# 3DAnimals/3DAnimals

Hardware: AMD Instinct MI355X
Metric: train images/sec fwd+bwd @256x256 b16 (higher is better)
Workload: dtype f32

## Files before the change

3danimals_amd/_lib.py:

```python
from __future__ import annotations

import ctypes
import os

import torch

_HERE = os.path.dirname(os.path.abspath(__file__))
LIB_PATH = os.environ.get("A3D_LIB") or os.path.join(_HERE, "lib", "liba3d_hip.so")

_c_int, _c_float, _c_size_t, _p = ctypes.c_int, ctypes.c_float, ctypes.c_size_t, ctypes.c_void_p

SIGNATURES = {
    "a3d_version": (_c_int, []),
    "a3d_last_error": (ctypes.c_char_p, []),
    "a3d_bw_probe_fill": (_c_int, [_p, ctypes.c_int64, _p]),
    "a3d_bw_probe_read": (_c_int, [_p, ctypes.c_int64, _p, _p]),
    "a3d_dmtet_scratch_bytes": (_c_size_t, [_c_int, _c_int]),
    "a3d_dmtet_count": (_c_int, [_p, _p, _p, _c_int, _c_int, _p, _p, _p, _c_int, _c_int, _p, _p, _c_int, _p, _c_int, _p]),
    "a3d_dmtet_count_ordered": (_c_int, [_p, _c_int, _c_int, _c_int, _p, _p, _p, _p, _c_int, _p, _c_int, _p]),
    "a3d_dmtet_word_group_slots": (_c_int, []),
    "a3d_dmtet_word_group_bits": (_c_int, []),
    "a3d_dmtet_block_items": (_c_int, []),
    "a3d_dmtet_vertex_scratch_bytes": (_c_size_t, [_c_int]),
    "a3d_dmtet_gather_rows": (_c_int, [_p, _p, ctypes.c_int64, ctypes.c_int64, _c_int, _p, _p]),
    "a3d_dmtet_emit": (_c_int, [_p, _p, _p, _p, _c_int, _c_int, _p, _c_int, _c_int, _c_int, _p, _p, _p, _p, _p, _p]),
    "a3d_dmtet_emit_sparse": (_c_int, [_p, _p, _p, _p, _c_int, _c_int, _p, _c_int, _c_int, _c_int, _p, _p, _p, _p, _p, _p]),
    "a3d_dmtet_bwd": (_c_int, [_p, _p, _p, _p, _p, _c_int, _c_int, _p, _p, _c_int, _p]),
    "a3d_skin_fwd": (_c_int, [_p, _c_int, _p, _c_int, _p, _c_int, _c_int, _c_int, _c_float, _p, _p, _p, _p]),
    "a3d_skin_bwd": (_c_int, [_p, _p, _c_int, _p, _c_int, _p, _c_int, _c_int, _c_int, _c_float, _p, _p, _c_int, _p]),
    "a3d_bone_transforms_fwd": (_c_int, [_p, _c_int, _p, _p, _c_int, _c_int, _c_int, _p, _p]),
    "a3d_bone_transforms_bwd": (_c_int, [_p, _p, _c_int, _p, _p, _c_int, _c_int, _c_int, _p, _p]),
    "a3d_estimate_bones": (_c_int, [_p, _p]),
    "a3d_skin_pose_max_bones": (_c_int, []),
    "a3d_skin_pose_products_floats": (_c_size_t, [_c_int, _c_int]),
    "a3d_skin_pose_fwd": (_c_int, [_p, _c_int, _p, _c_int, _p, _p, _c_int, _c_int, _c_int, _c_int, _c_float, _p, _p, _p, _p, _p]),
    "a3d_skin_pose_bwd": (_c_int, [_p, _p, _c_int, _p, _c_int, _p, _p, _p, _p, _c_int, _c_int, _c_int, _c_int, _c_float, _p, _p, _p, _c_int, _p]),
    "a3d_normals_adjacency": (_c_int, [_p, _c_int, _c_int, _p, _p, _p, _p]),
    "a3d_normals_fwd": (_c_int, [_p, _p, _p, _p, _c_int, _c_int, _c_int, _p, _p, _c_int, _p]),
    "a3d_normals_fwd_pair": (_c_int, [_p, _c_int, _p, _c_int, _p, _p, _p, _c_int, _c_int, _p, _p, _p, _p, _c_int, _p]),
    "a3d_normals_bwd": (_c_int, [_p, _c_int, _p, _p, _p, _p, _p, _c_int, _c_int, _c_int, _p, _p, _c_int, _p, _p]),
    "a3d_shade_fwd": (_c_int, [_p, _p, _c_int, _p, _p, _c_int, ctypes.c_int64, _c_int, _p, _p, _p, _p, _c_int, _p]),
    "a3d_shade_bwd": (_c_int, [_p, _p, _p, _p, _p, _c_int, _p, _c_int, _p, _c_int, ctypes.c_int64, _c_int, _p, _p, _p, _c_int, _p]),
    "a3d_shade_bwd_rows": (_c_int, [_p, _p, _p, _p, _p, ctypes.c_int64, _p, _c_int, ctypes.c_int64, _c_int, _p, _p, _c_int, ctypes.c_int64, _p]),
    "a3d_xfm_points_fwd": (_c_int, [_p, _c_int, _p, _c_int, _c_int, _c_int, _p, _p, _p]),
    "a3d_flow_delta_fwd": (_c_int, [_p, _c_int, _c_int, _c_int, _p, _p]),
    "a3d_flow_delta_bwd": (_c_int, [_p, _c_int, _p, _c_int, _c_int, _c_int, _p, _p]),
    "a3d_xfm_points_bwd": (_c_int, [_p, _c_int, _p, _c_int, _p, _c_int, _c_int, _c_int, _p, _p, _c_int, _p, _c_int, _p, _c_int, _p, _c_int, _p]),
    "a3d_cover_scratch_bytes": (_c_size_t, [_c_int, _c_int, _c_int]),
    "a3d_cover_blocks": (_c_int, [_c_int, _c_int, _c_int]),
    "a3d_cover_groups": (_c_int, [_c_int, _c_int, _c_int]),
    "a3d_cover_group_stride": (_c_int, []),
    "a3d_cover_count": (_c_int, [_p, _c_int, _c_int, _c_int, _c_int, _p, _p]),
    "a3d_cover_emit": (_c_int, [_p, _c_int, _c_int, _c_int, _c_int, _p, _p, _p, _p]),
    "a3d_rast_scratch_bytes": (_c_size_t, [_c_int, _c_int, _c_int]),
    "a3d_rast_bins_bytes": (_c_size_t, [_c_int, _c_int, _c_int, _c_int]),
    "a3d_rast_resolve": (_c_int, [_p, _c_int, _p, _c_int, _c_int, _c_int, _c_int, _c_int, _p, _p, _p, _p]),
    "a3d_rast_resolve_gbuffer_fwd": (_c_int, [_p, _c_int, _p, _c_int, _c_int, _c_int, _c_int, _c_int, _p, _p, _p, ctypes.c_int64, _p, _p, _p, _p, _p,
                                              _c_int, _p, _p, _c_int, _p, _p, _p, _p]),
    "a3d_rast_fwd": (_c_int, [_p, _c_int, _p, _c_int, _c_int, _c_int, _c_int, _c_int, _p, _p, _c_int, _p, _p]),
    "a3d_dispatch_order_probe": (_c_int, [_c_int, _c_int, _p, _p]),
    "a3d_rast_bwd": (_c_int, [_p, _p, _p, _c_int, _p, _c_int, _c_int, _c_int, _c_int, _c_int, _p, _p]),
    "a3d_interp_fwd": (_c_int, [_p, _c_int, _c_int, _p, _p, _c_int, _c_int, _c_int, _c_int, _c_int, _p, _p]),
    "a3d_interp_bwd": (_c_int, [_p, _p, _c_int, _c_int, _p, _p, _c_int, _c_int, _c_int, _c_int, _c_int, _p, _p, _p]),
    "a3d_mesh_topology": (_c_int, [_p, _c_int, _c_int, _p, _p, _p, _p, _p, _c_int, _p]),
    "a3d_mesh_topology_finalize_max_vertices": (_c_int, []),
    "a3d_mesh_topology_finalize": (_c_int, [_p, _c_int, _c_int, _p, _p, _p, _p, _c_int, _p]),
    "a3d_gbuffer_fwd": (_c_int, [_p, _p, _p, ctypes.c_int64, _p, _p, _p, _c_int, _c_int, _c_int, _c_int, _c_int, _c_int, _p, _p, _c_int, _p, _p, _p, _p]),
    "a3d_cover_gbuffer_fwd": (_c_int, [_p, _p, _c_int, _c_int, _c_int, _c_int, _c_int, _p, ctypes.c_int64, _p, _p, _p, _p, _p, _c_int, _p, _p, _c_int,
                                       _p, _p, _p, _p]),
    "a3d_gbuffer_bwd": (_c_int, [_p, _p, _p, _p, ctypes.c_int64, _p, _p, _p, _c_int, _p, _c_int, _c_int, _c_int, _c_int, _c_int, _p, _c_int,
                                 _c_int, _p, _c_int, _p, _p, _p]),
    "a3d_gbuffer_prior_grad": (_c_int, [_p, _c_int, _c_int, _p, _p]),
    "a3d_gemm_nn_relumask": (_c_int, [_p, _p, _p, ctypes.c_int64, _c_int, _c_int, _p, _p]),
    "a3d_harmonic_embed_fwd": (_c_int, [_p, _p, _c_int, _c_int, _c_int, ctypes.c_int64, _p, _p]),
    "a3d_harmonic_embed_bwd": (_c_int, [_p, _p, _p, _c_int, _c_int, _c_int, ctypes.c_int64, _p, _p]),
    "a3d_recon_losses_scratch_bytes": (_c_size_t, [_c_int, _c_int, _c_int]),
    "a3d_recon_losses_mask_bytes": (_c_size_t, [_c_int, _c_int, _c_int]),
    "a3d_recon_losses_columns": (_c_int, []),
    "a3d_recon_losses_fwd": (_c_int, [_p, _p, _c_int, _c_int, _p, _p, _p, _p, _p, ctypes.c_int64, _p, _c_int, _c_int, _c_int, _p, _p, _p, _p]),
    "a3d_recon_losses_bwd": (_c_int, [_p, _p, _p, _c_int, _c_int, _c_int, _p, _p, _p, _p, _p, ctypes.c_int64, _p, _c_int, _c_int, _c_int, _p, _p, _p, _p]),
    "a3d_flow_loss_scratch_bytes": (_c_size_t, [_c_int, _c_int, _c_int, _c_int]),
    "a3d_flow_loss_fwd": (_c_int, [_p, _c_int, _p, _p, _c_int, _c_int, _c_int, _c_int, _p, _p, _p, _p]),
    "a3d_flow_loss_bwd": (_c_int, [_p, _p, _p, _c_int, _p, _p, _c_int, _c_int, _c_int, _c_int, _p, _p]),
    "a3d_rows_segsum": (_c_int, [_p, _p, ctypes.c_int64, _c_int, _c_int, _p, _p]),
    "a3d_rows_add_relu_fwd": (_c_int, [_p, _p, _p, ctypes.c_int64, _c_int, _c_int, _p]),
    "a3d_rows_add_relu_bwd": (_c_int, [_p, _p, _p, ctypes.c_int64, _c_int, _c_int, _p, _p, _p]),
    "a3d_aa_hash_bytes": (_c_size_t, [_c_int]),
    "a3d_aa_shards": (_c_int, []),
    "a3d_aa_capacity": (_c_int, [_c_int, _c_int, _c_int]),
    "a3d_aa_topology": (_c_int, [_p, _c_int, _c_int, _p, _p, _p]),
    "a3d_aa_topology_from_lists": (_c_int, [_p, _c_int, _p, _p, _p, _c_int, _p]),
    "a3d_aa_analyze": (_c_int, [_p, _p, _c_int, _p, _p, _c_int, _c_int, _c_int, _c_int, _c_int, _p, _p, _c_int, _p, _c_int, _p, _p, _c_int, _p]),
    "a3d_aa_fwd": (_c_int, [_p, _c_int, _p, _p, _c_int, _c_int, _c_int, _c_int, _p, _p]),
    "a3d_aa_bwd": (_c_int, [_p, _p, _c_int, _p, _p, _c_int, _p, _c_int, _p, _c_int, _c_int, _c_int, _c_int, _c_int, _p, _p, _p]),
    "a3d_composite_aa_fwd": (_c_int, [_p, _p, _p, _p, _p, _c_int, _c_int, _c_int, _c_int, _p, _p, _p]),
    "a3d_mask_aa_fwd": (_c_int, [_p, _c_int, _p, _c_int, _p, _p, _p, _c_int, _c_int, _c_int, _c_int, _p, _p]),
    "a3d_mask_aa_bwd": (_c_int, [_p, _p, _c_int, _p, _c_int, _p, _p, _c_int, _p, _c_int, _p, _c_int, _c_int, _c_int, _c_int, _c_int, _p, _c_int, _p]),
    "a3d_composite_aa_bwd": (_c_int, [_p, _p, _p, ctypes.c_int64, _p, _p, _p, _c_int, _p, _c_int, _p, _c_int, _c_int, _c_int, _c_int, _c_int, _p, _p, _p]),
}



class DmtetOrder(ctypes.Structure):

    _fields_ = [("size", ctypes.c_uint32), ("group_slots", ctypes.c_int32), ("vertex_of_rank", _p), ("edges_ranked", _p), ("edge_of_row", _p),
                ("tets_ranked", _p), ("tet_of_row", _p), ("edge_groups", _p), ("tet_groups", _p)]


class RastOpts(ctypes.Structure):

    _fields_ = [("size", ctypes.c_uint32), ("lists_stride", ctypes.c_int32), ("prev_rast", _p), ("cover_scratch", _p), ("aa_screen", _p),
                ("aa_count", _p), ("topo_off", _p), ("topo_adj", _p), ("topo_opp", _p), ("normals_v_a", _p), ("normals_v_b", _p),
                ("normals_off", _p), ("normals_adj", _p), ("normals_acc_a", _p), ("normals_a", _p), ("normals_acc_b", _p), ("normals_b", _p),
                ("normals_B_a", ctypes.c_int32), ("normals_B_b", ctypes.c_int32), ("bins", _p), ("bin_cap", ctypes.c_int32), ("bins_clean", ctypes.c_int32),
                ("defer_resolve", ctypes.c_int32), ("reserved", ctypes.c_int32)]


class AaRide(ctypes.Structure):

    _fields_ = [("size", ctypes.c_uint32), ("clip_batch", ctypes.c_int32), ("rast", _p), ("screen", _p), ("tri", _p), ("opp", _p), ("off", _p),
                ("adj", _p), ("V", ctypes.c_int32), ("F", ctypes.c_int32), ("lists_stride", ctypes.c_int32), ("reserved", ctypes.c_int32)]


class CaBuffer(ctypes.Structure):

    _fields_ = [("size", ctypes.c_uint32), ("C", ctypes.c_int32), ("vals", _p), ("bg", _p), ("out", _p), ("g_out", _p), ("g_vals", _p),
# ... 346 lines not shown
```

3danimals_amd/csrc/build.py:

```python
import os
import subprocess
import sys
from concurrent.futures import ThreadPoolExecutor

HERE = os.path.dirname(os.path.abspath(__file__))
PKG = os.path.dirname(HERE)
LIB_DIR = os.path.join(PKG, "lib")
LIB = os.path.join(LIB_DIR, "liba3d_hip.so")
OBJ_DIR = os.path.join(HERE, "build")

SOURCES = {
    "common.hip": [],
    "dmtet.hip": ["-ffp-contract=off"],
    "skin.hip": [],
    "bones.hip": [],
    "normals.hip": ["-ffp-contract=off"],
    "raster.hip": ["-ffp-contract=off"],
    "cover.hip": [],
    "shade.hip": ["-ffp-contract=off"],
    "interp.hip": [],
    "gbuffer.hip": [],
    "segsum.hip": [],
    "losses.hip": [],
    "embed.hip": ["-ffp-contract=off"],
    "gemm.hip": [],
    "antialias.hip": ["-ffp-contract=off"],
    "topology.hip": [],
    "xfm.hip": ["-ffp-contract=off"],
}
COMMON = ["--offload-arch=gfx950", "-O3", "-std=c++17", "-fPIC", "-fhip-fp32-correctly-rounded-divide-sqrt", "-Wall",
          "-Wno-unused-function"]


def _hipcc():
    for c in (os.environ.get("HIPCC"), "/opt/rocm/bin/hipcc", "hipcc"):
        if c and (os.path.isabs(c) and os.path.exists(c) or not os.path.isabs(c)):
            return c
    raise RuntimeError("hipcc not found")


def _stale(target, deps):
    if not os.path.exists(target):
        return True
    t = os.path.getmtime(target)
    return any(os.path.getmtime(d) > t for d in deps)


def build(force=False, verbose=True, profile=False, exp=False):
    assert not (profile and exp)
    lib = os.path.join(LIB_DIR, "liba3d_hip_prof.so") if profile else (os.path.join(LIB_DIR, "liba3d_hip_exp.so") if exp else LIB)
    obj_dir = os.path.join(OBJ_DIR, "prof") if profile else (os.path.join(OBJ_DIR, "exp") if exp else OBJ_DIR)
    os.makedirs(LIB_DIR, exist_ok=True)
    os.makedirs(obj_dir, exist_ok=True)
    hipcc = _hipcc()
    headers = sorted(os.path.join(HERE, f) for f in os.listdir(HERE) if f.endswith(".h")) + [os.path.join(os.path.dirname(PKG), "include", "a3d.h"), os.path.abspath(__file__)]
    jobs = []
    objs = []
    for src, extra in SOURCES.items():
        s = os.path.join(HERE, src)
        o = os.path.join(obj_dir, src.replace(".hip", ".o"))
        objs.append(o)
        if force or _stale(o, [s] + headers):
            jobs.append([hipcc, "-x", "hip", "-c", s, "-o", o] + COMMON + extra + (["-DA3D_PROFILE"] if profile else []) + (["-DA3D_EXPERIMENT"] if exp else []))

    def run(cmd):
        if verbose:
            print(" ".join(cmd), flush=True)
        subprocess.check_call(cmd)

    with ThreadPoolExecutor(max_workers=min(8, max(1, len(jobs)))) as ex:
        list(ex.map(run, jobs))
    if force or jobs or _stale(lib, objs):
        run([hipcc, "--offload-arch=gfx950", "-shared", "-fPIC", "-o", lib] + objs)
    return lib


if __name__ == "__main__":
    print(build(force="--force" in sys.argv, profile="--profile" in sys.argv, exp="--exp" in sys.argv))
# ... 1 lines not shown
```

3danimals_amd/hostnets.py:

```python
from __future__ import annotations

import torch
import torch.nn as nn
import torch.nn.functional as F


REFERENCE_FORMULATION = False


def reference_formulation(enable=True):
    global REFERENCE_FORMULATION
    REFERENCE_FORMULATION = bool(enable)
    return REFERENCE_FORMULATION


def _activation(name):
    table = {"tanh": nn.Tanh, "sigmoid": nn.Sigmoid, "relu": nn.ReLU}
    if name not in table:
        raise NotImplementedError(name)
    return table[name]()


class HarmonicEmbedding(nn.Module):

# ... 61 lines not shown
        return y

    @staticmethod
    def backward(ctx, g):
        x, weight, y = ctx.saved_tensors
        g = torch.ops.aten.threshold_backward(g.contiguous(), y, 0)
        gx = g.mm(weight) if ctx.needs_input_grad[0] else None
        gw = _split_k_weight_grad(g, x) if ctx.needs_input_grad[1] else None
        gb = g.sum(0) if ctx.needs_input_grad[2] else None
        return gx, gw, gb


class _FieldStack(torch.autograd.Function):

    @staticmethod
    def forward(ctx, x_emb, w_in, per_image, index, w_first, *hidden):
        from . import ops

        zero = _zero_bias(x_emb, w_in)
        ys = [torch._addmm_activation(zero, x_emb, w_in.t(), use_gelu=False)]
        if w_first is not None:
            y = ys[0].mm(w_first.t())
            ops.rows_add_relu_raw_(y, per_image, index)
            ys.append(y)
        for w in hidden:
            ys.append(torch._addmm_activation(zero, ys[-1], w.t(), use_gelu=False))
        ctx.save_for_backward(x_emb, w_in, index, w_first, *hidden, *ys)
        ctx.n_hidden, ctx.n_images = len(hidden), (per_image.shape[0] if per_image is not None else 0)
        return ys[-1]

    @staticmethod
    @torch.autograd.function.once_differentiable
    def backward(ctx, g):
        from . import ops

        saved = ctx.saved_tensors
        x_emb, w_in, index, w_first = saved[:4]
        hidden, ys = saved[4:4 + ctx.n_hidden], saved[4 + ctx.n_hidden:]
        g = torch.ops.aten.threshold_backward(g.contiguous(), ys[-1], 0)
        g_hidden = []
        for i in range(ctx.n_hidden - 1, -1, -1):
            y_prev = ys[len(ys) - ctx.n_hidden - 1 + i]
            g_hidden.append(_split_k_weight_grad(g, y_prev))
            g = ops.gemm_nn_relumask(g, hidden[i], y_prev)
        g_hidden.reverse()
        g_rows = g_first = None
        if w_first is not None:
            g_rows = ops.rows_segsum_raw(g, index, ctx.n_images)
            g_first = _split_k_weight_grad(g, ys[0])
            g = ops.gemm_nn_relumask(g, w_first, ys[0])
        g_in = _split_k_weight_grad(g, x_emb)
        g_x = g.mm(w_in) if ctx.needs_input_grad[0] else None
        return (g_x, g_in, g_rows, None, g_first, *g_hidden)


def _long_list(x, weight):
    return (x.is_cuda and x.dim() == 2 and x.shape[0] >= SPLITK_MIN_ROWS and x.shape[0] % SPLITK_PARTS == 0 and x.is_contiguous()
            and x.dtype == torch.float32 and torch.is_grad_enabled() and weight.requires_grad)


def linear(x, weight, bias=None):
    if bias is None and _long_list(x, weight):
        return _LinearSplitK.apply(x, weight)
    return F.linear(x, weight, bias)


def linear_relu(x, weight, bias=None):
    if _long_list(x, weight):
        return _LinearReLUSplitK.apply(x, weight, bias)
    if (x.is_cuda and x.dim() == 2 and x.shape[0] >= SPLITK_MIN_ROWS and x.dtype == torch.float32
            and not (torch.is_grad_enabled() and (x.requires_grad or weight.requires_grad or (bias is not None and bias.requires_grad)))):
        return torch._addmm_activation(_zero_bias(x, weight) if bias is None else bias, x, weight.t(), use_gelu=False)
    return torch.relu_(F.linear(x, weight, bias))


class MLP(nn.Module):

    def __init__(self, cin, cout, num_layers, nf=256, dropout=0, activation=None):
        super().__init__()
        assert num_layers >= 1
        dims = [cin] + [nf] * (num_layers - 1) + [cout]
        layers = []
        for i in range(num_layers):
            if i > 0:
                layers.append(nn.ReLU(inplace=True))
            layers.append(nn.Linear(dims[i], dims[i + 1], bias=False))
            if dropout and 0 < i < num_layers - 1:
                layers.append(nn.Dropout(dropout))
        if activation is not None:
            layers.append(_activation(activation))
        self.network = nn.Sequential(*layers)

    def forward(self, x, first_weight=None, per_image=None, index=None):
        if REFERENCE_FORMULATION and first_weight is None:
            return self.network(x)
        layers = list(self.network)
        i = 0
        if first_weight is not None:
            assert isinstance(layers[0], nn.Linear) and layers[0].bias is None
            x = linear(x, first_weight)
            if len(layers) > 1 and isinstance(layers[1], nn.ReLU) and x.is_cuda:
                from . import ops

                x = ops.rows_add_relu_(x, per_image, index)
                i = 2
            else:
# ... 79 lines not shown
        if self.symmetrize:
            xs, ys, zs = x.unbind(-1)
            x = torch.stack([xs.abs(), ys, zs], -1)
        x_in = x
        if self.embedder is not None:
            x_in = self.embedder(x)
            if self.embed_concat_pts:
                x_in = torch.cat([x, x_in], -1)
        x_in = self.in_layer(x_in)
        if self.in_layer_relu:
            x_in = self.relu(x_in)
        if feat is not None:
            for _ in range(x_in.dim() - feat.dim()):
                feat = feat.unsqueeze(1)
            x_in = torch.cat([x_in, feat.expand(*x_in.shape[:-1], -1)], dim=-1)
        out = self.mlp(self.relu(x_in))
        if self.min_max is not None:
            out = out * (self.min_max[:, 1] - self.min_max[:, 0]) + self.min_max[:, 0]
        return out

    def _fused_input_ok(self, x):
        return (x.is_cuda and x.dim() == 2 and x.shape[1] == 3 and x.shape[0] >= SPLITK_MIN_ROWS and x.dtype == torch.float32
                and self.embedder is not None and self.embed_concat_pts and self.in_layer.bias is not None)

    def _fused_input(self, x):
        from . import ops

        h = ops.harmonic_embed(x, self.embedder._frequencies(x.device), symmetrize=self.symmetrize, ones=True)
        weight = torch.cat([self.in_layer.weight, self.in_layer.bias[:, None]], dim=1)
        return linear_relu(h, weight, None)

    def _stack_ok(self, x, with_feat):
        if not (USE_FIELD_STACK and self._fused_input_ok(x) and torch.is_grad_enabled() and x.shape[0] % SPLITK_PARTS == 0
                and self.in_layer.weight.requires_grad and self.in_layer.weight.shape[0] == 256):
            return False
        layers = list(self.mlp.network)
        n_pairs = 0
        while 2 * n_pairs + 1 < len(layers) and isinstance(layers[2 * n_pairs], nn.Linear) and isinstance(layers[2 * n_pairs + 1], nn.ReLU):
            lin = layers[2 * n_pairs]
            want_in = 256 + (self.extra_feat_dim if (with_feat and n_pairs == 0) else 0)
            if lin.bias is not None or tuple(lin.weight.shape) != (256, want_in):
                return False
            n_pairs += 1
        return n_pairs >= 1

    def _stacked(self, x, feat, feat_index):
        from . import ops

        layers = list(self.mlp.network)
        pairs, i = [], 0
        while i + 1 < len(layers) and isinstance(layers[i], nn.Linear) and isinstance(layers[i + 1], nn.ReLU):
            pairs.append(layers[i])
            i += 2
        x_emb = ops.harmonic_embed(x, self.embedder._frequencies(x.device), symmetrize=self.symmetrize, ones=True)
        w_in = torch.cat([self.in_layer.weight, self.in_layer.bias[:, None]], dim=1)
        if feat is not None:
            first = pairs[0].weight
            per_image = F.linear(torch.relu(feat), first[:, 256:])
            h = _FieldStack.apply(x_emb, w_in, per_image, feat_index, first[:, :256].contiguous(), *[l.weight for l in pairs[1:]])
        else:
            h = _FieldStack.apply(x_emb, w_in, None, None, None, *[l.weight for l in pairs])
        for layer in layers[i:]:
            h = linear(h, layer.weight, layer.bias) if isinstance(layer, nn.Linear) else layer(h)
        if self.min_max is not None:
            h = h * (self.min_max[:, 1] - self.min_max[:, 0]) + self.min_max[:, 0]
        return h

    def _forward_indexed(self, x, feat, feat_index):
        if self._stack_ok(x, True):
            return self._stacked(x, feat, feat_index)
        if self._fused_input_ok(x):
            h = self._fused_input(x)
        else:
            if self.symmetrize:
                x = torch.cat([x[..., :1].abs(), x[..., 1:]], -1)
            h = x
            if self.embedder is not None:
                h = self.embedder(x)
                if self.embed_concat_pts:
                    h = torch.cat([x, h], -1)
            h = linear_relu(h, self.in_layer.weight, self.in_layer.bias)
        nf = h.shape[-1]
        weight = self.mlp.network[0].weight
        per_image = F.linear(torch.relu(feat), weight[:, nf:])
        out = self.mlp(h, first_weight=weight[:, :nf].contiguous(), per_image=per_image, index=feat_index)
        if self.min_max is not None:
            out = out * (self.min_max[:, 1] - self.min_max[:, 0]) + self.min_max[:, 0]
        return out

    def sample(self, x, feat=None, feat_index=None):
        return self.forward(x, feat, feat_index)


class Linear_Mod(nn.Module):
    def __init__(self, in_features, out_features, bias=True):
        super().__init__()
        self.in_features, self.out_features = in_features, out_features
        self.weight = nn.Parameter(torch.empty((out_features, in_features)))
        if bias:
            self.bias = nn.Parameter(torch.empty(out_features))
        else:
            self.register_parameter("bias", None)
        nn.init.kaiming_uniform_(self.weight, a=5 ** 0.5)
        if self.bias is not None:
            fan_in, _ = nn.init._calculate_fan_in_and_fan_out(self.weight)
            bound = 1 / fan_in ** 0.5 if fan_in > 0 else 0
            nn.init.uniform_(self.bias, -bound, bound)

    def forward(self, x, style):
        if style.dim() > 1:
            style = style.reshape(-1, style.shape[-1])[0]
        weight = self.weight * style.unsqueeze(0)
        weight = weight / ((weight * weight).sum(dim=-1, keepdim=True) + 1e-5).sqrt()
        return F.linear(x, weight, self.bias)

# ... 64 lines not shown
```

3danimals_amd/ops.py:

```python
from __future__ import annotations

import ctypes
import math
import os
from collections import OrderedDict

import torch

from . import _lib
from ._lib import call, f32c, f32h, ptr, require_device, stream


class _IdentityCache:

    def __init__(self, maxsize=8):
        self.maxsize = maxsize
        self.data = OrderedDict()

    @staticmethod
    def key(t):
        return (t.data_ptr(), tuple(t.shape), t.dtype, t._version)

    def get(self, t, make):
        k = self.key(t)
# ... 1622 lines not shown
        ctx.save_for_backward(flow, flow_gt, both, scale)
        ctx.dims = (B, F, H, W)
        return loss

    @staticmethod
    def backward(ctx, g_loss):
        flow, flow_gt, both, scale = ctx.saved_tensors
        B, F, H, W = ctx.dims
        g_flow = torch.empty((B * F, H, W, 2), dtype=torch.float32, device=flow.device)
        call("a3d_flow_loss_bwd", ptr(f32h(g_loss)), ptr(scale), ptr(flow), flow.stride(2), ptr(flow_gt), ptr(both), B, F, H, W, ptr(g_flow), stream())
        return g_flow, None, None, None, None


def flow_loss(flow_nchw, flow_gt, both, batch, num_frames):
    return _FlowLoss.apply(flow_nchw.permute(0, 2, 3, 1), flow_gt, both, int(batch), int(num_frames))


class _HarmonicEmbed(torch.autograd.Function):
    @staticmethod
    def forward(ctx, x, freq, symmetrize, ones):
        require_device(x, freq, what="harmonic_embed")
        x, freq = f32c(x), f32c(freq)
        P, n = x.shape[0], freq.shape[0]
        assert x.shape == (P, 3)
        out = torch.empty((P, 3 + 6 * n + int(ones)), dtype=torch.float32, device=x.device)
        call("a3d_harmonic_embed_fwd", ptr(x), ptr(freq), n, int(symmetrize), int(ones), P, ptr(out), stream())
        ctx.save_for_backward(x, freq)
        ctx.cfg = (int(symmetrize), int(ones))
        return out

    @staticmethod
    @torch.autograd.function.once_differentiable
    def backward(ctx, g):
        x, freq = ctx.saved_tensors
        g_x = torch.empty_like(x)
        call("a3d_harmonic_embed_bwd", ptr(f32h(g)), ptr(x), ptr(freq), freq.shape[0], ctx.cfg[0], ctx.cfg[1], x.shape[0], ptr(g_x), stream())
        return g_x, None, None, None


def harmonic_embed(x, freq, symmetrize=False, ones=False):
    return _HarmonicEmbed.apply(x, freq, symmetrize, ones)


def gemm_nn_relumask(a, b, x=None):
    require_device(a, b, what="gemm_nn_relumask")
    a, b = f32c(a), f32c(b)
    M, K = a.shape
    assert b.shape == (K, 256) and K % 32 == 0 and (x is None or (x.shape == (M, 256) and x.is_contiguous() and x.dtype == torch.float32))
    c = torch.empty((M, 256), dtype=torch.float32, device=a.device)
    call("a3d_gemm_nn_relumask", ptr(a), ptr(b), ptr(x), M, 256, K, ptr(c), stream())
    return c


def _amp_wrap_functions():
    from torch.amp import custom_bwd, custom_fwd

    for obj in list(globals().values()):
        if isinstance(obj, type) and issubclass(obj, torch.autograd.Function) and obj is not torch.autograd.Function and obj.__module__ == __name__:
            obj.forward = staticmethod(custom_fwd(obj.forward, device_type="cuda", cast_inputs=torch.float32))
            obj.backward = staticmethod(custom_bwd(obj.backward, device_type="cuda"))


_amp_wrap_functions()

if _lib.GUARD:
    _lib.set_guard(_lib.GUARD)
```

include/a3d.h:

```cpp
#ifndef A3D_H
#define A3D_H
#include <stddef.h>
#include <stdint.h>

#ifdef __cplusplus
extern "C" {
#endif

#define A3D_OK 0
#define A3D_EINVAL (-1)
#define A3D_EHIP (-2)

typedef void* a3d_stream_t;

int a3d_version(void);
const char* a3d_last_error(void);

int a3d_bw_probe_fill(float* dst, int64_t n_floats, a3d_stream_t stream);
int a3d_bw_probe_read(const float* src, int64_t n_floats, float* sink, a3d_stream_t stream);

size_t a3d_dmtet_scratch_bytes(int Ne, int Nt);
int a3d_dmtet_count(const float* sdf, const int32_t* edges, const int32_t* tets, int Ne, int Nt, void* scratch,
                    int32_t* counts , void* vertex_scratch_or_null, int vertex_scratch_is_clean, int Nv,
                    const uint32_t* edge_groups_or_null, const uint32_t* tet_groups_or_null, int group_slots ,
// ... 227 lines not shown
    const int32_t* tri;
    const int32_t* opp;
    const int32_t* off;
    const int32_t* adj;
    int32_t V;
    int32_t F;
    int32_t lists_stride;
    int32_t reserved;
} a3d_aa_ride;
typedef struct a3d_ca_shade {
    uint32_t size;
    int32_t kd_stride;
    const float* gb;
    const float* par;
    const float* kd;
    float* clear;
    int32_t n_clear;
    int32_t two_sided;
    const a3d_shade_params* params;
    float* shaded_out;
} a3d_ca_shade;
typedef struct a3d_ca_buffer {
    uint32_t size;
    int32_t C;
    const float* vals;
    const float* bg;
    float* out;
    const float* g_out;
    float* g_vals;
    int32_t bg_batch;
    int32_t reserved;
    int32_t bg_channels;
    int32_t g_stride;
    int32_t g_channels;
    int32_t out_channels;
    int64_t vals_rows;
} a3d_ca_buffer;
int a3d_composite_aa_fwd(const a3d_ca_buffer* first, const a3d_ca_buffer* second_or_null, const int32_t* inv, void* work, int32_t* count,
                         int capacity, int B, int H, int W, const a3d_aa_ride* analyze_or_null, const a3d_ca_shade* shade_or_null,
                         a3d_stream_t stream);
int a3d_mask_aa_fwd(const float* rast, int C, const float* bg_or_null, int bg_batch, float* out, void* work, int32_t* count, int capacity,
                    int B, int H, int W, const a3d_aa_ride* analyze_or_null , a3d_stream_t stream);
int a3d_mask_aa_bwd(const float* g_out, const float* rast, int C, const float* bg_or_null, int bg_batch, const void* work,
                    const int32_t* count, int capacity, const float* clip, int clip_batch, const int32_t* tri, int B, int V, int F, int H,
                    int W, float* g_clip,
                    int g_channels_first ,
                    a3d_stream_t stream);
int a3d_composite_aa_bwd(const a3d_ca_buffer* first, const a3d_ca_buffer* second_or_null, const int64_t* pix, int64_t P, const int32_t* inv,
                         const void* work, const int32_t* count, int capacity, const float* clip, int clip_batch, const int32_t* tri, int B,
                         int V, int F, int H, int W, float* g_clip, const a3d_ca_shade* shade_or_null, a3d_stream_t stream);

int a3d_gemm_nn_relumask(const float* A, const float* B, const float* X, int64_t M, int N, int K, float* C, a3d_stream_t stream);

int a3d_harmonic_embed_fwd(const float* x , const float* freq , int n, int symmetrize, int ones, int64_t P, float* out,
                           a3d_stream_t stream);
int a3d_harmonic_embed_bwd(const float* g_out, const float* x, const float* freq, int n, int symmetrize, int ones, int64_t P, float* g_x,
                           a3d_stream_t stream);

size_t a3d_recon_losses_scratch_bytes(int B, int H, int W);
size_t a3d_recon_losses_mask_bytes(int B, int H, int W);
int a3d_recon_losses_columns(void);
int a3d_recon_losses_fwd(const float* shaded, const float* dino, int D, int dino_stride, const float* image_gt, const float* dino_gt, const float* mask_gt,
                         const float* dt0, const float* dt1_or_null, int64_t dt_stride, const float* valid, int B, int H, int W, void* scratch,
                         uint8_t* both, float* loss, a3d_stream_t stream);
int a3d_recon_losses_bwd(const float* g_loss, const float* shaded, const float* dino, int D, int dino_stride, int g_dino_stride, const float* image_gt, const float* dino_gt,
                         const float* mask_gt, const float* dt0, const float* dt1_or_null, int64_t dt_stride, const float* valid, int B, int H,
                         int W, const uint8_t* both, float* g_shaded, float* g_dino, a3d_stream_t stream);
size_t a3d_flow_loss_scratch_bytes(int B, int F, int H, int W);
int a3d_flow_loss_fwd(const float* flow, int pix_stride, const float* flow_gt, const uint8_t* both, int B, int F, int H, int W, void* scratch,
                      float* loss, float* scale, a3d_stream_t stream);
int a3d_flow_loss_bwd(const float* g_loss, const float* scale, const float* flow, int pix_stride, const float* flow_gt, const uint8_t* both,
                      int B, int F, int H, int W, float* g_flow, a3d_stream_t stream);

int a3d_xfm_points_fwd(const float* points, int points_batch, const float* matrix, int matrix_batch, int B, int V, float* out,
                       float* g_matrix_to_clear_or_null, a3d_stream_t stream);
int a3d_xfm_points_bwd(const float* g_out, int g_stride, const float* points, int points_batch, const float* matrix, int matrix_batch, int B, int V,
                       float* g_points_or_null, float* g_matrix_or_null, int g_matrix_is_clear,
                       const float* g_points_addend_or_null ,
                       int addend_stride,
                       const float* g_points_addend2_or_null ,
                       int addend2_stride,
                       const float* g_out2_or_null ,
                       int g2_stride, a3d_stream_t stream);
int a3d_flow_delta_fwd(const float* clip, int N, int F, int V, float* delta, a3d_stream_t stream);
int a3d_flow_delta_bwd(const float* g_delta, int g_stride , const float* clip, int N,
                       int F, int V, float* g_clip, a3d_stream_t stream);

#ifdef __cplusplus
}
#endif
#endif
```

Baseline: 1044.

## Fuse field MLP head and input-layer backward into custom HIP kernels

```diff
diff --git a/3danimals_amd/_lib.py b/3danimals_amd/_lib.py
--- a/3danimals_amd/_lib.py
+++ b/3danimals_amd/_lib.py
@@ -72,6 +72,9 @@
                                  _c_int, _p, _c_int, _p, _p, _p]),
     "a3d_gbuffer_prior_grad": (_c_int, [_p, _c_int, _c_int, _p, _p]),
     "a3d_gemm_nn_relumask": (_c_int, [_p, _p, _p, ctypes.c_int64, _c_int, _c_int, _p, _p]),
+    "a3d_field_workspace_floats": (_c_size_t, [_c_int, _c_int]),
+    "a3d_field_head_bwd": (_c_int, [_p, _p, _p, ctypes.c_int64, _c_int, _p, _p, _p, ctypes.c_int64, _p]),
+    "a3d_field_input_bwd": (_c_int, [_p, _p, _p, _p, _p, ctypes.c_int64, _c_int, _c_int, _c_int, _p, _p, _p, ctypes.c_int64, _p]),
     "a3d_harmonic_embed_fwd": (_c_int, [_p, _p, _c_int, _c_int, _c_int, ctypes.c_int64, _p, _p]),
     "a3d_harmonic_embed_bwd": (_c_int, [_p, _p, _p, _c_int, _c_int, _c_int, ctypes.c_int64, _p, _p]),
     "a3d_recon_losses_scratch_bytes": (_c_size_t, [_c_int, _c_int, _c_int]),
diff --git a/3danimals_amd/csrc/build.py b/3danimals_amd/csrc/build.py
--- a/3danimals_amd/csrc/build.py
+++ b/3danimals_amd/csrc/build.py
@@ -24,6 +24,7 @@
     "losses.hip": [],
     "embed.hip": ["-ffp-contract=off"],
     "gemm.hip": [],
+    "field_bwd.hip": [],
     "antialias.hip": ["-ffp-contract=off"],
     "topology.hip": [],
     "xfm.hip": ["-ffp-contract=off"],
diff --git a/3danimals_amd/csrc/field_bwd.hip b/3danimals_amd/csrc/field_bwd.hip
--- /dev/null
+++ b/3danimals_amd/csrc/field_bwd.hip
@@ -0,0 +1,315 @@
+#include "a3d_common.h"
+
+namespace {
+
+typedef float f32x16 __attribute__((ext_vector_type(16)));
+typedef float f32x4 __attribute__((ext_vector_type(4)));
+
+constexpr int FB_N = 256;
+
+constexpr int HB_WAVES = 8;
+
+template <int C>
+__global__ __launch_bounds__(64 * HB_WAVES, 2) void fh_bwd_kernel(const float* __restrict__ g_out, const float* __restrict__ y,
+                                                                   const float* __restrict__ w, int M, float* __restrict__ g_l,
+                                                                   float* __restrict__ slab) {
+    constexpr int HB_ROWS = C > 8 ? 2 : 4;
+    __shared__ f32x4 red[HB_WAVES / 2][C][64];
+    const int lane = threadIdx.x & 63;
+    const int wave = __builtin_amdgcn_readfirstlane(threadIdx.x >> 6);
+    f32x4 wr[C], acc[C];
+#pragma unroll
+    for (int c = 0; c < C; ++c) {
+        wr[c] = *reinterpret_cast<const f32x4*>(w + c * FB_N + 4 * lane);
+        acc[c] = f32x4{0.f, 0.f, 0.f, 0.f};
+    }
+    const int n_groups = (M + HB_ROWS - 1) / HB_ROWS;
+    const int stride = gridDim.x * HB_WAVES;
+    for (int gi = blockIdx.x * HB_WAVES + wave; gi < n_groups; gi += stride) {
+        const int m0 = gi * HB_ROWS;
+        f32x4 yv[HB_ROWS];
+        float gv[HB_ROWS][C];
+#pragma unroll
+        for (int r = 0; r < HB_ROWS; ++r) {
+            const int m = m0 + r < M ? m0 + r : M - 1;
+            yv[r] = *reinterpret_cast<const f32x4*>(y + (long long)m * FB_N + 4 * lane);
+#pragma unroll
+            for (int c = 0; c < C; ++c) gv[r][c] = m0 + r < M ? g_out[(long long)m * C + c] : 0.f;
+        }
+#pragma unroll
+        for (int r = 0; r < HB_ROWS; ++r) {
+            f32x4 s = {0.f, 0.f, 0.f, 0.f};
+#pragma unroll
+            for (int c = 0; c < C; ++c) {
+                s += gv[r][c] * wr[c];
+                acc[c] += gv[r][c] * yv[r];
+            }
+            if (m0 + r < M) {
+                f32x4 o;
+                o.x = yv[r].x > 0.f ? s.x : 0.f;
+                o.y = yv[r].y > 0.f ? s.y : 0.f;
+                o.z = yv[r].z > 0.f ? s.z : 0.f;
+                o.w = yv[r].w > 0.f ? s.w : 0.f;
+                *reinterpret_cast<f32x4*>(g_l + (long long)(m0 + r) * FB_N + 4 * lane) = o;
+            }
+        }
+    }
+#pragma unroll
+    for (int h = HB_WAVES / 2; h >= 1; h >>= 1) {
+        __syncthreads();
+        if (wave >= h && wave < 2 * h)
+#pragma unroll
+            for (int c = 0; c < C; ++c) red[wave - h][c][lane] = acc[c];
+        __syncthreads();
+        if (wave < h)
+#pragma unroll
+            for (int c = 0; c < C; ++c) acc[c] += red[wave][c][lane];
+    }
+    if (wave == 0)
+#pragma unroll
+        for (int c = 0; c < C; ++c) *reinterpret_cast<f32x4*>(slab + ((long long)blockIdx.x * C + c) * FB_N + 4 * lane) = acc[c];
+}
+
+constexpr int IB_WAVES = 8, IB_KP = 64;
+
+template <bool GX>
+__global__ __launch_bounds__(64 * IB_WAVES, 1) void fi_bwd_kernel(const float* __restrict__ g0, const float* __restrict__ xe,
+                                                                  const float* __restrict__ x, const float* __restrict__ freq,
+                                                                  const float* __restrict__ w, int M, int K, int n, int symmetrize,
+                                                                  float* __restrict__ g_x, float* __restrict__ slab) {
+    __shared__ float lds[2 * 4 * 32 * IB_KP];
+    const int tid = threadIdx.x, lane = tid & 63;
+    const int wave = __builtin_amdgcn_readfirstlane(tid >> 6), q = wave & 3, tm = wave >> 2;
+    const int row = lane & 31, kh = lane >> 5;
+    const int nq = 64 * q;
+
+    float wr[GX ? 8 : 1][4][2];
+    if (GX) {
+#pragma unroll
+        for (int g = 0; g < 8; ++g)
+#pragma unroll
+            for (int u = 0; u < 4; ++u)
+#pragma unroll
+                for (int b = 0; b < 2; ++b) {
+                    const int k = 32 * b + row;
+                    wr[g][u][b] = k < K ? w[(nq + 8 * g + 4 * kh + u) * K + k] : 0.f;
+                }
+    }
+    f32x16 wacc[2][2];
+#pragma unroll
+    for (int a = 0; a < 2; ++a)
+#pragma unroll
+        for (int b = 0; b < 2; ++b)
+#pragma unroll
+            for (int r = 0; r < 16; ++r) wacc[a][b][r] = 0.f;
+
+    const int n_tiles = (M + 31) >> 5;
+    const int stride = 2 * gridDim.x;
+    const int iters = (n_tiles + stride - 1) / stride;
+    for (int it = 0; it < iters; ++it) {
+        const int t = it * stride + 2 * blockIdx.x + tm;
+        const bool live = t < n_tiles;
+        const int m0 = 32 * t;
+        if (live) {
+            constexpr int PF = GX ? 8 : 16;
+            float ga[16][2], xb[16][2];
+            auto load_pair = [&](int p) {
+                const int m = m0 + 2 * p + kh;
+                const int mc = m < M ? m : M - 1;
+                const float* gp = g0 + (long long)mc * FB_N + nq + row;
+                const float* xp = xe + (long long)mc * K + row;
+#pragma unroll
+                for (int a = 0; a < 2; ++a) ga[p][a] = gp[32 * a];
+#pragma unroll
+                for (int b = 0; b < 2; ++b) xb[p][b] = (m < M && 32 * b + row < K) ? xp[32 * b] : 0.f;
+            };
+#pragma unroll
+            for (int p = 0; p < PF; ++p) load_pair(p);
+            if (GX) {
+                const int mr = m0 + row < M ? m0 + row : M - 1;
+                const float* a_lane = g0 + (long long)mr * FB_N + nq + 4 * kh;
+                f32x4 av[8];
+#pragma unroll
+                for (int g = 0; g < 8; ++g) av[g] = *reinterpret_cast<const f32x4*>(a_lane + 8 * g);
+                f32x16 tacc[2];
+#pragma unroll
+                for (int b = 0; b < 2; ++b)
+#pragma unroll
+                    for (int r = 0; r < 16; ++r) tacc[b][r] = 0.f;
+#pragma unroll
+                for (int g = 0; g < 8; ++g)
+#pragma unroll
+                    for (int u = 0; u < 4; ++u)
+#pragma unroll
+                        for (int b = 0; b < 2; ++b) tacc[b] = __builtin_amdgcn_mfma_f32_32x32x2f32(av[g][u], wr[g][u][b], tacc[b], 0, 0, 0);
+                float* tp = lds + (tm * 4 + q) * 32 * IB_KP;
+#pragma unroll
+                for (int b = 0; b < 2; ++b)
+#pragma unroll
+                    for (int r = 0; r < 16; ++r) tp[((r & 3) + 8 * (r >> 2) + 4 * kh) * IB_KP + 32 * b + row] = tacc[b][r];
+            }
+#pragma unroll
+            for (int p = PF; p < 16; ++p) load_pair(p);
+#pragma unroll
+            for (int p = 0; p < 16; ++p)
+#pragma unroll
+                for (int a = 0; a < 2; ++a)
+#pragma unroll
+                    for (int b = 0; b < 2; ++b) wacc[a][b] = __builtin_amdgcn_mfma_f32_32x32x2f32(ga[p][a], xb[p][b], wacc[a][b], 0, 0, 0);
+        }
+        if (GX) {
+            __syncthreads();
+            const int tt = tid & 255;
+            if (live && tt < 96) {
+                const int rr = tt / 3, c = tt - 3 * rr, m = m0 + rr;
+                if (m < M) {
+                    const float* tq = lds + (tm * 4 * 32 + rr) * IB_KP;
+                    constexpr int QS = 32 * IB_KP;
+                    const float* xr = xe + (long long)m * K;
+                    float acc = ((tq[c] + tq[QS + c]) + tq[2 * QS + c]) + tq[3 * QS + c];
+                    for (int k = 0; k < n; ++k) {
+                        const int js = 3 + c * n + k, jc = js + 3 * n;
+                        const float ts = ((tq[js] + tq[QS + js]) + tq[2 * QS + js]) + tq[3 * QS + js];
+                        const float tc = ((tq[jc] + tq[QS + jc]) + tq[2 * QS + jc]) + tq[3 * QS + jc];
+                        acc += freq[k] * (ts * xr[jc] - tc * xr[js]);
+                    }
+                    if (symmetrize && c == 0) {
+                        const float raw = x[3ll * m];
+                        acc *= raw > 0.f ? 1.f : (raw < 0.f ? -1.f : 0.f);
+                    }
+                    g_x[3ll * m + c] = acc;
+                }
+            }
+            __syncthreads();
+        }
+    }
+    __syncthreads();
+    float* wl = lds + q * (4 * 16 * 64);
+    if (tm == 1) {
+#pragma unroll
+        for (int a = 0; a < 2; ++a)
+#pragma unroll
+            for (int b = 0; b < 2; ++b)
+#pragma unroll
+                for (int r = 0; r < 16; ++r) wl[((2 * a + b) * 16 + r) * 64 + lane] = wacc[a][b][r];
+    }
+    __syncthreads();
+    if (tm == 0) {
+        float* sp = slab + (long long)blockIdx.x * FB_N * IB_KP;
+#pragma unroll
+        for (int a = 0; a < 2; ++a)
+#pragma unroll
+            for (int b = 0; b < 2; ++b)
+#pragma unroll
+                for (int r = 0; r < 16; ++r) {
+                    const int nn = nq + 32 * a + (r & 3) + 8 * (r >> 2) + 4 * kh, k = 32 * b + row;
+                    sp[nn * IB_KP + k] = wacc[a][b][r] + wl[((2 * a + b) * 16 + r) * 64 + lane];
+                }
+    }
+}
+
+__global__ __launch_bounds__(256) void fb_slab_sum_kernel(const float* __restrict__ slab, int S, int R, int K, int KS, float* __restrict__ out) {
+    __shared__ float part[16][17];
+    const int el = threadIdx.x & 15, ph = threadIdx.x >> 4;
+    const int e = blockIdx.x * 16 + el;
+    const bool ok = e < R * K;
+    float s = 0.f;
+    if (ok) {
+        const int r = e / K, k = e - r * K;
+        const float* p = slab + (long long)r * KS + k;
+        const long long ss = (long long)R * KS;
+        for (int i = ph; i < S; i += 16) s += p[i * ss];
+    }
+    part[ph][el] = s;
+    __syncthreads();
+    if (ph == 0 && ok) {
+        float t = 0.f;
+#pragma unroll
+        for (int i = 0; i < 16; ++i) t += part[i][el];
+        out[e] = t;
+    }
+}
+
+int fb_cu_count(int* n_cu) {
+    static int n_cu_of[64] = {0};
+    int dev = 0;
+    A3D_HIP(hipGetDevice(&dev));
+    A3D_CHECK_ARG(dev >= 0 && dev < 64);
+    if (!n_cu_of[dev]) {
+        int n = 0;
+        A3D_HIP(hipDeviceGetAttribute(&n, hipDeviceAttributeMultiprocessorCount, dev));
+        n_cu_of[dev] = n > 0 ? n : 1;
+    }
+    *n_cu = n_cu_of[dev];
+    return A3D_OK;
+}
+
+template <int C>
+void fh_launch(int grid, hipStream_t s, const float* g_out, const float* y, const float* w, int M, float* g_l, float* slab) {
+    hipLaunchKernelGGL(fh_bwd_kernel<C>, dim3(grid), dim3(64 * HB_WAVES), 0, s, g_out, y, w, M, g_l, slab);
+}
+
+}
+
+extern "C" size_t a3d_field_workspace_floats(int C, int K) {
+    int n_cu = 0;
+    if (fb_cu_count(&n_cu) != A3D_OK) return 0;
+    const size_t head = C > 0 ? (size_t)2 * n_cu * C * FB_N : 0;
+    const size_t in = K > 0 ? (size_t)n_cu * FB_N * IB_KP : 0;
+    return head > in ? head : in;
+}
+
+extern "C" int a3d_field_head_bwd(const float* g_out, const float* y, const float* w, int64_t M, int C, float* g_l, float* g_w,
+                                  float* work, int64_t work_floats, a3d_stream_t stream) {
+    A3D_CHECK_ARG(M >= 0 && M < 0x7fffffffll && C >= 1 && C <= 16);
+    hipStream_t s = (hipStream_t)stream;
+    A3D_CHECK_ARG(w && g_w);
+    if (M == 0) {
+        A3D_HIP(hipMemsetAsync(g_w, 0, sizeof(float) * C * FB_N, s));
+        return A3D_OK;
+    }
+    A3D_CHECK_ARG(g_out && y && g_l && work);
+    int n_cu = 0;
+    const int rc = fb_cu_count(&n_cu);
+    if (rc != A3D_OK) return rc;
+    const int grid = 2 * n_cu;
+    A3D_CHECK_ARG(work_floats >= (int64_t)grid * C * FB_N);
+    const int m = (int)M;
+    switch (C) {
+#define A3D_FH_CASE(c) \
+    case c: fh_launch<c>(grid, s, g_out, y, w, m, g_l, work); break;
+        A3D_FH_CASE(1) A3D_FH_CASE(2) A3D_FH_CASE(3) A3D_FH_CASE(4) A3D_FH_CASE(5) A3D_FH_CASE(6) A3D_FH_CASE(7) A3D_FH_CASE(8)
+        A3D_FH_CASE(9) A3D_FH_CASE(10) A3D_FH_CASE(11) A3D_FH_CASE(12) A3D_FH_CASE(13) A3D_FH_CASE(14) A3D_FH_CASE(15) A3D_FH_CASE(16)
+#undef A3D_FH_CASE
+    }
+    A3D_LAUNCH_CHECK();
+    hipLaunchKernelGGL(fb_slab_sum_kernel, dim3(a3d_div_up((long long)C * FB_N, 16)), dim3(256), 0, s, work, grid, C, FB_N, FB_N, g_w);
+    A3D_LAUNCH_CHECK();
+    return A3D_OK;
+}
+
+extern "C" int a3d_field_input_bwd(const float* g0, const float* x_emb, const float* x, const float* freq, const float* w_in, int64_t M,
+                                   int K, int n, int symmetrize, float* g_w, float* g_x, float* work, int64_t work_floats,
+                                   a3d_stream_t stream) {
+    A3D_CHECK_ARG(M >= 0 && M < 0x7fffffffll && n >= 1 && K == 3 + 6 * n + 1 && K <= IB_KP);
+    hipStream_t s = (hipStream_t)stream;
+    A3D_CHECK_ARG(w_in && g_w);
+    if (M == 0) {
+        A3D_HIP(hipMemsetAsync(g_w, 0, sizeof(float) * FB_N * K, s));
+        return A3D_OK;
+    }
+    A3D_CHECK_ARG(g0 && x_emb && work && (g_x == nullptr || (x && freq)));
+    int n_cu = 0;
+    const int rc = fb_cu_count(&n_cu);
+    if (rc != A3D_OK) return rc;
+    const int grid = n_cu;
+    A3D_CHECK_ARG(work_floats >= (int64_t)grid * FB_N * IB_KP);
+    if (g_x)
+        hipLaunchKernelGGL(fi_bwd_kernel<true>, dim3(grid), dim3(64 * IB_WAVES), 0, s, g0, x_emb, x, freq, w_in, (int)M, K, n, symmetrize, g_x, work);
+    else
+        hipLaunchKernelGGL(fi_bwd_kernel<false>, dim3(grid), dim3(64 * IB_WAVES), 0, s, g0, x_emb, x, freq, w_in, (int)M, K, n, symmetrize, g_x, work);
+    A3D_LAUNCH_CHECK();
+    hipLaunchKernelGGL(fb_slab_sum_kernel, dim3(a3d_div_up((long long)FB_N * K, 16)), dim3(256), 0, s, work, grid, FB_N, K, IB_KP, g_w);
+    A3D_LAUNCH_CHECK();
+    return A3D_OK;
+}
diff --git a/3danimals_amd/hostnets.py b/3danimals_amd/hostnets.py
--- a/3danimals_amd/hostnets.py
+++ b/3danimals_amd/hostnets.py
@@ -137,6 +137,52 @@
         g_in = _split_k_weight_grad(g, x_emb)
         g_x = g.mm(w_in) if ctx.needs_input_grad[0] else None
         return (g_x, g_in, g_rows, None, g_first, *g_hidden)
+
+
+FUSED_FIELD_EDGES = True
+
+
+class _FieldStackEdges(torch.autograd.Function):
+
+    @staticmethod
+    def forward(ctx, x, x_emb, freq, symmetrize, w_in, per_image, index, w_first, w_head, *hidden):
+        from . import ops
+
+        zero = _zero_bias(x_emb, w_in)
+        ys = [torch._addmm_activation(zero, x_emb, w_in.t(), use_gelu=False)]
+        if w_first is not None:
+            y = ys[0].mm(w_first.t())
+            ops.rows_add_relu_raw_(y, per_image, index)
+            ys.append(y)
+        for w in hidden:
+            ys.append(torch._addmm_activation(zero, ys[-1], w.t(), use_gelu=False))
+        out = ys[-1].mm(w_head.t())
+        ctx.save_for_backward(x, x_emb, freq, w_in, index, w_first, w_head, *hidden, *ys)
+        ctx.n_hidden, ctx.n_images, ctx.symmetrize = len(hidden), (per_image.shape[0] if per_image is not None else 0), bool(symmetrize)
+        return out
+
+    @staticmethod
+    @torch.autograd.function.once_differentiable
+    def backward(ctx, g_out):
+        from . import ops
+
+        saved = ctx.saved_tensors
+        x, x_emb, freq, w_in, index, w_first, w_head = saved[:7]
+        hidden, ys = saved[7:7 + ctx.n_hidden], saved[7 + ctx.n_hidden:]
+        g, g_head = ops.field_head_bwd(g_out, ys[-1], w_head)
+        g_hidden = []
+        for i in range(ctx.n_hidden - 1, -1, -1):
+            y_prev = ys[len(ys) - ctx.n_hidden - 1 + i]
+            g_hidden.append(_split_k_weight_grad(g, y_prev))
+            g = ops.gemm_nn_relumask(g, hidden[i], y_prev)
+        g_hidden.reverse()
+        g_rows = g_first = None
+        if w_first is not None:
+            g_rows = ops.rows_segsum_raw(g, index, ctx.n_images)
+            g_first = _split_k_weight_grad(g, ys[0])
+            g = ops.gemm_nn_relumask(g, w_first, ys[0])
+        g_in, g_x = ops.field_input_bwd(g, x_emb, x, freq, w_in, ctx.symmetrize, want_gx=ctx.needs_input_grad[0])
+        return (g_x, None, None, None, g_in, g_rows, None, g_first, g_head, *g_hidden)
 
 
 def _long_list(x, weight):
@@ -322,6 +368,10 @@
         while i + 1 < len(layers) and isinstance(layers[i], nn.Linear) and isinstance(layers[i + 1], nn.ReLU):
             pairs.append(layers[i])
             i += 2
+        head = layers[i] if i < len(layers) else None
+        if (FUSED_FIELD_EDGES and isinstance(head, nn.Linear) and head.bias is None and head.weight.shape[0] <= 16
+                and tuple(head.weight.shape[1:]) == (256,) and head.weight.requires_grad):
+            return self._stacked_edges(x, feat, feat_index, pairs, head, layers[i + 1:])
         x_emb = ops.harmonic_embed(x, self.embedder._frequencies(x.device), symmetrize=self.symmetrize, ones=True)
         w_in = torch.cat([self.in_layer.weight, self.in_layer.bias[:, None]], dim=1)
         if feat is not None:
@@ -331,6 +381,25 @@
         else:
             h = _FieldStack.apply(x_emb, w_in, None, None, None, *[l.weight for l in pairs])
         for layer in layers[i:]:
+            h = linear(h, layer.weight, layer.bias) if isinstance(layer, nn.Linear) else layer(h)
+        if self.min_max is not None:
+            h = h * (self.min_max[:, 1] - self.min_max[:, 0]) + self.min_max[:, 0]
+        return h
+
+    def _stacked_edges(self, x, feat, feat_index, pairs, head, rest):
+        from . import ops
+
+        freq = self.embedder._frequencies(x.device)
+        x_emb = ops.harmonic_embed_raw(x, freq, symmetrize=self.symmetrize, ones=True)
+        w_in = torch.cat([self.in_layer.weight, self.in_layer.bias[:, None]], dim=1)
+        if feat is not None:
+            first = pairs[0].weight
+            per_image = F.linear(torch.relu(feat), first[:, 256:])
+            h = _FieldStackEdges.apply(x, x_emb, freq, self.symmetrize, w_in, per_image, feat_index, first[:, :256].contiguous(), head.weight,
+                                       *[l.weight for l in pairs[1:]])
+        else:
+            h = _FieldStackEdges.apply(x, x_emb, freq, self.symmetrize, w_in, None, None, None, head.weight, *[l.weight for l in pairs])
+        for layer in rest:
             h = linear(h, layer.weight, layer.bias) if isinstance(layer, nn.Linear) else layer(h)
         if self.min_max is not None:
             h = h * (self.min_max[:, 1] - self.min_max[:, 0]) + self.min_max[:, 0]
diff --git a/3danimals_amd/ops.py b/3danimals_amd/ops.py
--- a/3danimals_amd/ops.py
+++ b/3danimals_amd/ops.py
@@ -1698,6 +1698,49 @@
     return c
 
 
+def harmonic_embed_raw(x, freq, symmetrize=False, ones=False):
+    require_device(x, freq, what="harmonic_embed")
+    x, freq = f32c(x), f32c(freq)
+    P, n = x.shape[0], freq.shape[0]
+    assert x.shape == (P, 3)
+    out = torch.empty((P, 3 + 6 * n + int(ones)), dtype=torch.float32, device=x.device)
+    call("a3d_harmonic_embed_fwd", ptr(x), ptr(freq), n, int(symmetrize), int(ones), P, ptr(out), stream())
+    return out
+
+
+def _field_work(c, k, device):
+    n = _lib.lib().a3d_field_workspace_floats(c, k)
+    if n <= 0:
+        raise _lib.A3DError(f"a3d_field_workspace_floats failed: {_lib.lib().a3d_last_error().decode()}")
+    return torch.empty(n, dtype=torch.float32, device=device)
+
+
+def field_head_bwd(g_out, y, w):
+    require_device(g_out, y, w, what="field_head_bwd")
+    g_out, w = f32c(g_out), f32c(w)
+    M, C = g_out.shape
+    assert w.shape == (C, 256) and 1 <= C <= 16 and y.shape == (M, 256) and y.is_contiguous() and y.dtype == torch.float32
+    g_l = torch.empty((M, 256), dtype=torch.float32, device=y.device)
+    g_w = torch.empty((C, 256), dtype=torch.float32, device=y.device)
+    work = _field_work(C, 0, y.device)
+    call("a3d_field_head_bwd", ptr(g_out), ptr(y), ptr(w), M, C, ptr(g_l), ptr(g_w), ptr(work), work.numel(), stream(), tag=f"[C{C}]")
+    return g_l, g_w
+
+
+def field_input_bwd(g0, x_emb, x, freq, w_in, symmetrize=False, want_gx=True):
+    require_device(g0, x_emb, x, freq, w_in, what="field_input_bwd")
+    g0, x_emb, x, freq, w_in = f32c(g0), f32c(x_emb), f32c(x), f32c(freq), f32c(w_in)
+    M, K = x_emb.shape
+    n = freq.shape[0]
+    assert g0.shape == (M, 256) and x.shape == (M, 3) and w_in.shape == (256, K) and K == 3 + 6 * n + 1 and K <= 64
+    g_w = torch.empty((256, K), dtype=torch.float32, device=g0.device)
+    g_x = torch.empty((M, 3), dtype=torch.float32, device=g0.device) if want_gx else None
+    work = _field_work(0, K, g0.device)
+    call("a3d_field_input_bwd", ptr(g0), ptr(x_emb), ptr(x), ptr(freq), ptr(w_in), M, K, n, int(symmetrize), ptr(g_w), ptr(g_x), ptr(work),
+         work.numel(), stream(), tag=f"[K{K}]")
+    return g_w, g_x
+
+
 def _amp_wrap_functions():
     from torch.amp import custom_bwd, custom_fwd
 
diff --git a/include/a3d.h b/include/a3d.h
--- a/include/a3d.h
+++ b/include/a3d.h
@@ -303,6 +303,12 @@
 
 int a3d_gemm_nn_relumask(const float* A, const float* B, const float* X, int64_t M, int N, int K, float* C, a3d_stream_t stream);
 
+size_t a3d_field_workspace_floats(int C, int K);
+int a3d_field_head_bwd(const float* g_out, const float* y, const float* w, int64_t M, int C, float* g_l, float* g_w, float* work,
+                       int64_t work_floats, a3d_stream_t stream);
+int a3d_field_input_bwd(const float* g0, const float* x_emb, const float* x, const float* freq, const float* w_in, int64_t M, int K, int n,
+                        int symmetrize, float* g_w, float* g_x, float* work, int64_t work_floats, a3d_stream_t stream);
+
 int a3d_harmonic_embed_fwd(const float* x , const float* freq , int n, int symmetrize, int ones, int64_t P, float* out,
                            a3d_stream_t stream);
 int a3d_harmonic_embed_bwd(const float* g_out, const float* x, const float* freq, int n, int symmetrize, int ones, int64_t P, float* g_x,
```

Result: no change. 1064 (median of 6 runs) (+1.9%).
